# barry-mir/mixing-style-transfer

Hardware: AMD Instinct MI355X
Metric: triplets/sec (10 s @ 44.1 kHz, 4-stem, bs=24) (higher is better)
Workload: dtype f32

## Files before the change

include/mst.h:

```cpp
#ifndef MST_H_
#define MST_H_

#include <stddef.h>
#include <stdint.h>

#ifdef __cplusplus
extern "C" {
#endif

#define MST_ABI_VERSION 1

#define MST_OK 0
#define MST_EINVAL (-1)
#define MST_ENOMEM (-2)
#define MST_EHIP (-3)

int mst_version(void);
const char* mst_last_error(void);

typedef struct mst_plan mst_plan;

int mst_plan_create(mst_plan** out, int sample_rate, int n_fft, int hop, int n_mels,
                    const float* window, const float* fb, int detailed_bins);
void mst_plan_destroy(mst_plan* plan);
// ... 69 lines not shown
int mst_encoder_forward(const mst_encoder* enc, const float* logmel, int frames, const float* feats,
                        int B, float* emb, const mst_encoder_taps* taps, void* workspace,
                        size_t workspace_bytes, void* stream);

typedef struct mst_logmel_in {
  int32_t layout;
  int32_t pad_;
  const void* data;
  const void* lo;
  const uint32_t* absmax;
} mst_logmel_in;
int mst_encoder_layout_supported(const mst_encoder* enc, int layout);
int mst_encoder_forward_in(const mst_encoder* enc, const mst_logmel_in* logmel, int frames, const float* feats,
                           int B, float* emb, const mst_encoder_taps* taps, void* workspace,
                           size_t workspace_bytes, void* stream);

typedef struct mst_encoder_train_taps {
  float* film;
  float* pool1;
  float* pool_in;
  float* bn1;
  float* bn2;
  const float* film_in;
  const unsigned char* drop1_mask;
  float drop1_scale;
  int phase;
  double count_scale;
  unsigned char* drop1_mask_out;
  uint64_t drop1_seed;
  float drop1_p;
// ... 294 lines not shown
```

mixing-style-transfer_amd/_lib.py:

```python
import ctypes as C
import os
import subprocess
import threading

_HERE = os.path.dirname(os.path.abspath(__file__))
LIB_PATH = os.environ.get("MST_LIB", os.path.join(_HERE, "libmst.so"))
CSRC = os.path.join(_HERE, "csrc")

MST_OK = 0


class MstError(RuntimeError):
    pass


class EncoderConfig(C.Structure):
    _fields_ = [("n_mels", C.c_int32), ("split_size", C.c_int32), ("overlap", C.c_int32),
                ("n_subbands", C.c_int32), ("feature_dim", C.c_int32), ("embed_dim", C.c_int32),
                ("film_hidden", C.c_int32), ("attn_hidden", C.c_int32), ("bn_eps", C.c_float)]


_W_FIELDS = ["conv1_w", "conv1_b", "bn1_w", "bn1_b", "bn1_mean", "bn1_var",
             "conv2_w", "conv2_b", "bn2_w", "bn2_b", "bn2_mean", "bn2_var",
             "mlp0_w", "mlp0_b", "mlp3_w", "mlp3_b", "head_w", "head_b",
# ... 125 lines not shown
    "mst_melfeat_forward_stems_pcm16": (C.c_int, [C.c_void_p, C.POINTER(C.c_void_p), C.c_longlong, C.c_int, C.c_int,
                                                  C.c_void_p, C.c_void_p, C.c_void_p, C.c_size_t, C.c_void_p]),
    "mst_plan_layout_supported": (C.c_int, [C.c_void_p, C.c_int]),
    "mst_melfeat_forward_io": (C.c_int, [C.c_void_p, C.POINTER(MelfeatIO), C.c_int, C.c_int, C.c_void_p, C.c_size_t,
                                         C.c_void_p]),
    "mst_encoder_layout_supported": (C.c_int, [C.c_void_p, C.c_int]),
    "mst_encoder_forward_in": (C.c_int, [C.c_void_p, C.POINTER(LogmelIn), C.c_int, C.c_void_p, C.c_int, C.c_void_p,
                                         C.POINTER(EncoderTaps), C.c_void_p, C.c_size_t, C.c_void_p]),
    "mst_encoder_create": (C.c_int, [C.POINTER(C.c_void_p), C.POINTER(EncoderConfig), C.POINTER(EncoderWeights)]),
    "mst_encoder_destroy": (None, [C.c_void_p]),
    "mst_encoder_set_precision": (C.c_int, [C.c_void_p, C.c_int]),
    "mst_encoder_set_train_precision": (C.c_int, [C.c_void_p, C.c_int]),
    "mst_encoder_workspace_bytes": (C.c_size_t, [C.c_void_p, C.c_int, C.c_int]),
    "mst_encoder_forward": (C.c_int, [C.c_void_p, C.c_void_p, C.c_int, C.c_void_p, C.c_int, C.c_void_p,
                                      C.POINTER(EncoderTaps), C.c_void_p, C.c_size_t, C.c_void_p]),
    "mst_encoder_train_workspace_bytes": (C.c_size_t, [C.c_void_p, C.c_int, C.c_int]),
    "mst_encoder_forward_train": (C.c_int, [C.c_void_p, C.c_void_p, C.c_int, C.c_void_p, C.c_int, C.c_void_p,
                                            C.POINTER(EncoderTrainTaps), C.c_void_p, C.c_size_t, C.c_void_p]),
    "mst_dropout_mask": (C.c_int, [C.c_float, C.c_uint64, C.c_longlong, C.c_void_p, C.c_void_p]),
    "mst_head_save_bytes": (C.c_size_t, [C.POINTER(HeadDims), C.c_int, C.c_float]),
    "mst_head_backward_workspace_bytes": (C.c_size_t, [C.POINTER(HeadDims), C.c_int]),
    "mst_head_forward_train": (C.c_int, [C.POINTER(HeadDims), C.POINTER(HeadPtrs), C.c_void_p, C.c_int, C.c_float, C.c_uint64, C.c_float,
                                         C.c_uint64, C.c_void_p, C.c_void_p, C.c_size_t, C.c_void_p]),
    "mst_head_backward": (C.c_int, [C.POINTER(HeadDims), C.POINTER(HeadPtrs), C.c_void_p, C.c_int, C.c_float, C.c_uint64, C.c_float,
                                    C.c_uint64, C.c_void_p, C.c_void_p, C.POINTER(HeadPtrs), C.c_void_p, C.c_void_p, C.c_size_t, C.c_void_p]),
    "mst_film_save_bytes": (C.c_size_t, [C.POINTER(FilmDims), C.c_int]),
    "mst_film_backward_workspace_bytes": (C.c_size_t, [C.POINTER(FilmDims), C.c_int]),
    "mst_film_forward_train": (C.c_int, [C.POINTER(FilmDims), C.POINTER(FilmPtrs), C.c_void_p, C.c_int, C.c_float, C.c_uint64,
                                         C.c_void_p, C.c_void_p, C.c_size_t, C.c_void_p]),
    "mst_film_backward": (C.c_int, [C.POINTER(FilmDims), C.POINTER(FilmPtrs), C.c_void_p, C.c_int, C.c_float, C.c_void_p, C.c_void_p,
# ... 165 lines not shown
```

mixing-style-transfer_amd/csrc/encoder.hip:

```cpp
#include "common.h"

#include <cmath>
#include <type_traits>
#include <vector>

namespace {

typedef float f32x4 __attribute__((ext_vector_type(4)));
constexpr int kConvThreads = 512;
constexpr int kConvWaves = 8;

struct FilmParams {
  const float* feats;
  const float *w0t, *b0, *w3t, *b3, *hwt, *hb;
  const float *s1, *t1, *s2, *t2;
  float* film;
  float2* aff1;
  float2* aff2;
  int Fd, H, nsub;
  float* h2;
  int B;
};

constexpr int kFilmCT = 8;
// ... 87 lines not shown
  }
  __syncthreads();
  for (int idx = tid; idx < kFilmCT * 32; idx += 256) {
    const int c = idx >> 5, ch = idx & 31, b = b0 + c;
    if (b >= p.B) continue;
    const float g = fl[c * 64 + ch], be = fl[c * 64 + 32 + ch];
    if (slice == 0) {
      p.aff1[((size_t)b * p.nsub + band) * 32 + ch] = make_float2(g * p.s1[band * 32 + ch], fmaf(g, p.t1[band * 32 + ch], be));
    } else {
      const int c2 = 32 * (slice - 1) + ch;
      p.aff2[((size_t)b * p.nsub + band) * 64 + c2] = make_float2(g * p.s2[band * 64 + c2], fmaf(g, p.t2[band * 64 + c2], be));
    }
  }
}

constexpr size_t film_lds_bytes(int Fd, int H) {
  return (size_t)((Fd + H) * kFilmCT + 5 * kFilmCT * 64) * sizeof(float);
}
hipError_t launch_film(const FilmParams& fp, hipStream_t st) {
  const int tiles = (fp.B + kFilmCT - 1) / kFilmCT;
  const size_t lds_h = (size_t)((fp.Fd + fp.H) * kFilmCT + 4 * kFilmCT * 64) * sizeof(float);
  const size_t lds_o = (size_t)(fp.H * kFilmCT + 5 * kFilmCT * 64) * sizeof(float);
  hipLaunchKernelGGL(film_hidden_kernel, dim3(tiles, (fp.H + 63) / 64), dim3(256), lds_h, st, fp);
  hipLaunchKernelGGL(film_head_kernel, dim3(tiles, fp.nsub * 3), dim3(256), lds_o, st, fp);
  return hipGetLastError();
}

template <int LAYER, int SUB>
struct CC;
template <int SUB>
struct CC<1, SUB> {
  static constexpr int CIN = 8, COUT = 32, NCH = 2, MT = 5, NT = 2;
  static constexpr int WIN = 5 * SUB;
  static constexpr int WPG = 20 / WIN;
  static constexpr int TROWS = SUB, TCOLS = 5 * 4 * WPG;
  static constexpr int PR = TROWS + 6, PC = TCOLS + 6;
  static constexpr int RL = PC <= 64 ? 64 : 128;
};
template <int SUB>
// ... 2115 lines not shown
      for (int w = 0; w < 4; ++w)
        q4[w] = w == wave ? own[n][r] : red[((size_t)(wave * 3 + (w < wave ? w : w - 1)) * kAttnNT + n) * 256 + r * 64 + lane];
      part[r] = fmaf(w2, tanhf((q4[0] + q4[1]) + (q4[2] + q4[3]) + b1), part[r]);
    }
  }
#pragma unroll
  for (int r = 0; r < 4; ++r) {
    float v = part[r];
#pragma unroll
    for (int o = 8; o > 0; o >>= 1) v += __shfl_xor(v, o, 64);
    const int m = (mb * kAttnMT + wave) * 16 + 4 * kq + r;
    if (i == 0 && m < M) p.part[(size_t)nh * M + m] = v;
  }
}

struct PoolParams {
  const float* x;
  const float* part;
  const float* b2;
  float* pooled;
  int C, W;
  long long M;
};

__global__ __launch_bounds__(256) void attn_pool_kernel(const PoolParams p) {
  extern __shared__ float sm[];
  float* w = sm;
  __shared__ float red[8];
  const int b = blockIdx.x, tid = threadIdx.x, lane = tid & 63, wave = tid >> 6;
  const float b2 = p.b2[0];
// ... 62 lines not shown
#pragma unroll
    for (int u = 0; u < kProjU; ++u) acc = __builtin_amdgcn_mfma_f32_16x16x4f32(a[u], bb[u], acc, 0, 0, 0);
  }
#pragma unroll
  for (int r = 0; r < 4; ++r) red[wave][r][lane] = acc[r];
  __syncthreads();
  if (wave < 4) {
    const int e = nt * 16 + i, m = m0 + 4 * kq + wave;
    float v = 0.f;
#pragma unroll
    for (int w = 0; w < 8; ++w) v += red[w][wave][lane];
    if (m < p.B) p.emb[(size_t)m * p.E + e] = fmaxf(v + p.bias[e], 0.f);
  }
}

hipError_t launch_attn_scores(const AttnParams& ap, hipStream_t st) {
  const int mblocks = (ap.B * ap.W + 16 * kAttnMT - 1) / (16 * kAttnMT);
  return mst::launch_lds<attn_scores_kernel>(dim3(mblocks, kAttnHalves), dim3(256), kAttnLds, st, ap);
}

void launch_proj(const ProjParams& pj, hipStream_t st) {
  hipLaunchKernelGGL(proj_kernel, dim3(pj.E / 16, (pj.B + 15) / 16), dim3(512), 0, st, pj);
}

}

constexpr int kGenCols = 8, kGenPC = 5 * kGenCols + 6;
constexpr size_t conv1_generic_lds(int split_size) {
  return (size_t)(392 * 32 + 8 * (split_size + 6) * kGenPC) * sizeof(float);
}
__global__ __launch_bounds__(256) void conv1_generic_kernel(const ConvParams p, int sub) {
  extern __shared__ __attribute__((aligned(16))) float gsm[];
  float* wl = gsm;
  float* patch = gsm + 392 * 32;
  const int tid = threadIdx.x, co = tid & 31, pwl = tid >> 5;
  const int clip = blockIdx.y / p.nsub, band = blockIdx.y - clip * p.nsub;
  const int pw0 = blockIdx.x * kGenCols, PR = p.in_rows + 6;
// ... 1088 lines not shown
  p.in_clipstride = (long long)8 * e->cfg.n_mels * frames;
}
template <class P>
void conv2_input_geometry(P& p, const mst_encoder* e, int W1) {
  p.in_rows = e->H1, p.in_cols = W1;
  p.in_cstride = e->H1 * W1;
  p.in_bandoff = 32 * e->H1 * W1;
  p.in_clipstride = (long long)e->cfg.n_subbands * 32 * e->H1 * W1;
}

FilmParams film_params(const mst_encoder* e, const float* feats, float* film, float2* aff1, float2* aff2, float* h2, int B) {
  return FilmParams{feats, e->w0t, e->b0, e->w3t, e->b3, e->hwt, e->hb, e->s1, e->t1, e->s2, e->t2,
                    film, aff1, aff2, e->cfg.feature_dim, e->cfg.film_hidden, e->cfg.n_subbands, h2, B};
}

int launch_head(const mst_encoder* e, const WsLayout& L, char* ws, const float* pool_in, float* emb, int B, hipStream_t st,
                void* scored = nullptr) {
  float* scores = reinterpret_cast<float*>(ws + L.scores);
  AttnParams ap{pool_in, e->att0frag, e->att0_b, e->att2_w, scores, B, e->C, L.W2, e->cfg.attn_hidden};
  MST_HIP_CHECK(launch_attn_scores(ap, st));
  if (scored) (void)hipEventRecord(reinterpret_cast<hipEvent_t>(scored), st);
  float* pooled = reinterpret_cast<float*>(ws + L.pooled);
  PoolParams pp{pool_in, scores, e->att2_b, pooled, e->C, L.W2, (long long)B * L.W2};
  const int slices = (e->C + 127) / 128;
  hipLaunchKernelGGL(attn_pool_kernel, dim3(B, slices), dim3(256), (size_t)((L.W2 + 3) & ~3) * sizeof(float), st, pp);
  MST_HIP_CHECK(hipGetLastError());
  ProjParams pj{pooled, e->projfrag, e->proj_b, emb, B, e->C, e->cfg.embed_dim};
  launch_proj(pj, st);
  MST_HIP_CHECK(hipGetLastError());
  return MST_OK;
}

#ifdef MST_TRACE
struct ConvTrace {
  float* buf = nullptr;
  int calls = 0;
};
void trace_attach(ConvTrace& t, ConvParams& cp) {
  if (!t.buf) (void)hipMalloc(&t.buf, 256 * kConvWaves * 8 * sizeof(float));
  cp.yraw = t.buf;
}
void trace_dump(ConvTrace& t, int g, bool conv2) {
  if (++t.calls != 10) return;
  (void)hipDeviceSynchronize();
  std::vector<float> h(256 * kConvWaves * 8);
// ... 121 lines not shown
}

static bool conv1_resident_geometry(const mst_encoder* e) {
  return (e->sub == 2 || (e->sub == 1 && e->cfg.split_size % 2 == 0)) && !getenv("MST_CONV1_CHUNKED");
}

int mst_encoder_layout_supported(const mst_encoder* e, int layout) {
  if (!e) return 0;
  if (layout == MST_LOGMEL_REF) return 1;
  if (e->sub > 2) return 0;
  if (layout == MST_LOGMEL_CM32) return e->conv1_f16x3 == 0 && conv1_resident_geometry(e);
  if (layout == MST_LOGMEL_CM16) return e->conv1_f16x3 != 0;
  return 0;
}

int mst_encoder_forward(const mst_encoder* e, const float* logmel, int frames, const float* feats, int B, float* emb,
                        const mst_encoder_taps* taps, void* workspace, size_t workspace_bytes, void* stream) {
  mst_logmel_in in{};
  in.layout = MST_LOGMEL_REF, in.data = logmel;
  return mst_encoder_forward_in(e, &in, frames, feats, B, emb, taps, workspace, workspace_bytes, stream);
}

int mst_encoder_forward_in(const mst_encoder* e, const mst_logmel_in* lin, int frames, const float* feats, int B, float* emb,
                           const mst_encoder_taps* taps, void* workspace, size_t workspace_bytes, void* stream) {
  MST_REQUIRE(e && lin && lin->data && feats && emb, "mst_encoder_forward: NULL argument");
  const int lay = lin->layout;
  if (const int rc = check_logmel_in("mst_encoder_forward", lin, mst_encoder_layout_supported(e, lay), e->conv1_f16x3,
                                     e->conv1_f16x3 != 3, e->conv1_f16x3 >= 2))
    return rc;
  const float* logmel = static_cast<const float*>(lin->data);
// ... 1006 lines not shown
```

mixing-style-transfer_amd/csrc/infonce.hip:

```cpp
#include "common.h"

namespace {

__global__ __launch_bounds__(256) void l2norm_kernel(const float* emb, float* inv_norm, int D) {
  __shared__ float red[4];
  const int r = blockIdx.x, tid = threadIdx.x;
  float a = 0.f;
  for (int d = tid; d < D; d += 256) {
    const float v = emb[(size_t)r * D + d];
    a = fmaf(v, v, a);
  }
  a = mst::wave_sum(a);
  if ((tid & 63) == 0) red[tid >> 6] = a;
  __syncthreads();
  if (tid == 0) inv_norm[r] = 1.0f / fmaxf(sqrtf((red[0] + red[1]) + (red[2] + red[3])), 1e-12f);
}

constexpr int kInfoThreads = 512, kInfoWaves = kInfoThreads / 64;
__global__ __launch_bounds__(kInfoThreads) void infonce_fwd_kernel(const float* __restrict__ emb, const int64_t* __restrict__ labels,
                                                                   float* sim, int N, int D, int row0, float inv_tau, float* rowout) {
  extern __shared__ float srow[];
  __shared__ float red[3 * kInfoWaves];
  const int i = row0 + blockIdx.x, tid = threadIdx.x, lane = tid & 63, wave = tid >> 6;
  auto inv_of = [](float sumsq) { return 1.0f / fmaxf(sqrtf(sumsq), 1e-12f); };
  {
    float q = 0.f;
    for (int d = lane; d < D; d += 64) {
      const float v = emb[(size_t)i * D + d];
      q = fmaf(v, v, q);
    }
    const float ni = inv_of(mst::wave_sum(q));
    for (int d = tid; d < D; d += kInfoThreads) srow[d] = emb[(size_t)i * D + d] * ni;
  }
  __syncthreads();
  float* s = sim + (size_t)blockIdx.x * N;
  float mx = -INFINITY;
  for (int j0 = wave * 4; j0 < N; j0 += 4 * kInfoWaves) {
    float a[4] = {0.f, 0.f, 0.f, 0.f}, q[4] = {0.f, 0.f, 0.f, 0.f};
    const float* ej[4];
#pragma unroll
    for (int u = 0; u < 4; ++u) ej[u] = emb + (size_t)min(j0 + u, N - 1) * D;
#pragma unroll 4
    for (int d = lane; d < D; d += 64) {
      const float x = srow[d];
#pragma unroll
      for (int u = 0; u < 4; ++u) {
        const float v = ej[u][d];
        a[u] = fmaf(x, v, a[u]);
        q[u] = fmaf(v, v, q[u]);
      }
    }
#pragma unroll
    for (int u = 0; u < 4; ++u) {
      const int j = j0 + u;
      if (j >= N) break;
      const float v = mst::wave_sum(a[u]) * inv_of(mst::wave_sum(q[u])) * inv_tau;
      if (lane == 0) s[j] = v;
// ... 146 lines not shown
  return mst::align_up((size_t)N * sizeof(float), 256) + mst::align_up((size_t)N * N * sizeof(float), 256) +
         mst::align_up((size_t)2 * N * sizeof(float), 256);
}

int mst_infonce_forward(const float* emb, const int64_t* labels, int N, int D, int row0, int rows, float temperature,
                        float* out, void* workspace, size_t workspace_bytes, void* stream) {
  MST_REQUIRE(emb && labels && out, "mst_infonce_forward: NULL argument");
  MST_REQUIRE(N > 0 && D > 0 && row0 >= 0 && rows > 0 && row0 + rows <= N && temperature > 0.f,
              "mst_infonce_forward: bad sizes N=%d D=%d row0=%d rows=%d", N, D, row0, rows);
  const size_t need = mst_infonce_workspace_bytes(N, D);
  if (!workspace || workspace_bytes < need)
    return mst::fail(MST_ENOMEM, "mst_infonce_forward: workspace %zu B < required %zu B", workspace_bytes, need);
  hipStream_t st = reinterpret_cast<hipStream_t>(stream);
  float* sim = reinterpret_cast<float*>(reinterpret_cast<char*>(workspace) + mst::align_up((size_t)N * sizeof(float), 256));
  float* rowout = reinterpret_cast<float*>(reinterpret_cast<char*>(sim) + mst::align_up((size_t)N * N * sizeof(float), 256));
  hipLaunchKernelGGL(infonce_fwd_kernel, dim3(rows), dim3(kInfoThreads), (size_t)D * sizeof(float), st, emb, labels, sim, N, D, row0,
                     1.0f / temperature, rowout);
  hipLaunchKernelGGL(infonce_reduce_kernel, dim3(1), dim3(256), 0, st, rowout, rows, out);
  MST_HIP_CHECK(hipGetLastError());
  return MST_OK;
}

int mst_infonce_backward(const float* emb, const int64_t* labels, int N, int D, int row0, int rows, float temperature,
                         const float* scale, float* grad, void* workspace, size_t workspace_bytes, void* stream) {
  MST_REQUIRE(emb && labels && grad, "mst_infonce_backward: NULL argument");
  MST_REQUIRE(N > 0 && D > 0 && row0 >= 0 && rows > 0 && row0 + rows <= N && temperature > 0.f,
              "mst_infonce_backward: bad sizes N=%d D=%d row0=%d rows=%d", N, D, row0, rows);
  const size_t coef_lds = (size_t)((D + 1) & ~1) * sizeof(float) + (size_t)N * sizeof(double);
  MST_REQUIRE(coef_lds <= 64 * 1024, "mst_infonce_backward: 4 D + 8 N = %zu B of LDS, limit 65536 (N=%d D=%d)", coef_lds, N, D);
  const size_t need = mst_infonce_workspace_bytes(N, D);
  if (!workspace || workspace_bytes < need)
    return mst::fail(MST_ENOMEM, "mst_infonce_backward: workspace %zu B < required %zu B", workspace_bytes, need);
// ... 13 lines not shown
```

mixing-style-transfer_amd/csrc/melfeat.hip:

```cpp
#include "common.h"
#include "fft_wave.h"
#include "fft_pk.h"
#include "stage_a_tables.h"

#include <algorithm>
#include <cmath>
#include <memory>
#include <vector>


namespace {

constexpr int kWaves = 8;
constexpr int kFPW = 2;
constexpr int kTF = kWaves * kFPW;
constexpr int kTileStride = kTF + 1;
constexpr int kThreads = kWaves * 64;
constexpr int nf_of(int n_fft) { return n_fft >= 2048 ? 1 : kFPW; }
constexpr int kNumScalars = 80;

enum : int {
  S_LOGSUM = 0,
  S_LINSUM = 4,
  S_MASK = 8,
// ... 814 lines not shown
  double sxy = 0, sxx = 0, syy = 0;
  for (int i = lane; i < n; i += 64) {
    const double dx = i - mx, dy = y[i] - my;
    sxy += dx * dy, sxx += dx * dx, syy += dy * dy;
  }
  sxy = wave_sum_f64(sxy), sxx = wave_sum_f64(sxx), syy = wave_sum_f64(syy);
  const double std_unbiased = sqrt(syy / (n - 1));
  if (std_unbiased < 1e-6) return 0.0;
  double c = sxy / sqrt(sxx * syy);
  return fmin(1.0, fmax(-1.0, c));
}

struct FinalizeLds {
  static constexpr int a_sc = 0, a_chmean = a_sc + kNumScalars * 8, a_chm2 = a_chmean + 64, a_cross = a_chm2 + 64, a_curve = a_cross + 64;
  static constexpr size_t bytes(int M, int detailed_bins) { return (size_t)4 * M * 8 + a_curve + (size_t)4 * (detailed_bins > 0 ? detailed_bins : 0) * 8; }
};

__global__ __launch_bounds__(256) void melfeat_finalize_kernel(const FParams p) {
  extern __shared__ __attribute__((aligned(16))) unsigned char smem[];
  using L = FinalizeLds;
  double* band = reinterpret_cast<double*>(smem);
  unsigned char* after_band = reinterpret_cast<unsigned char*>(band + 4 * p.M);
  double* sc = reinterpret_cast<double*>(after_band + L::a_sc);
  double* chmean = reinterpret_cast<double*>(after_band + L::a_chmean);
  double* chm2 = reinterpret_cast<double*>(after_band + L::a_chm2);
  double* cross = reinterpret_cast<double*>(after_band + L::a_cross);
  const int tid = threadIdx.x, clip = blockIdx.x, M = p.M;
  const float* base = p.partials + (size_t)clip * p.runs_per_clip * p.pstride;
  const double inv_n_db = 1.0 / (2.0 * p.F);
  const double k_db = 10.0 / log(10.0);
  for (int i = tid; i < 4 * M; i += 256) {
    double s = 0;
#pragma unroll 8
    for (int r = 0; r < p.runs_per_clip; ++r) s += base[(size_t)r * p.pstride + i];
    band[i] = s * inv_n_db * k_db;
  }
  if (tid < kNumScalars) {
    const bool is_max = tid >= S_PEAK && tid < S_PEAK + 8;
    double s = 0;
#pragma unroll 8
    for (int r = 0; r < p.runs_per_clip; ++r) {
      const double v = base[(size_t)r * p.pstride + 4 * M + tid];
      s = is_max ? fmax(s, v) : s + v;
    }
    sc[tid] = s;
  }
  if (tid < 8) {
    double n = 0, mean = 0, m2 = 0;
    for (int r = 0; r < p.runs_per_clip; ++r) {
      const float* q = base + (size_t)r * p.pstride + 4 * M;
      const double nr = q[S_NSAMP];
      if (nr <= 0) continue;
      const double sr = q[S_DSUM + tid], qr = q[S_DSQ + tid];
      const double mr = q[S_PIVOT + tid] + sr / nr, m2r = fmax(0.0, qr - sr * sr / nr);
      const double d = mr - mean, nt = n + nr;
      m2 += m2r + d * d * n * nr / nt;
      mean += d * nr / nt;
      n = nt;
    }
    chmean[tid] = mean, chm2[tid] = m2;
  } else if (tid >= 64 && tid < 68) {
    const int s = tid - 64;
// ... 333 lines not shown
    MST_HIP_CHECK(hipMemsetAsync(lmo.absmax, 0, (size_t)B * sizeof(unsigned), st));
  }
  const int runs = use_sw ? sw_runs(p, F) : runs_per_clip(p, F);
  auto common = [&](auto k) {
    for (int i = 0; i < 4; ++i) k.stem[i] = stems4[i];
    k.clip_stride = clip_stride, k.logmel = logmel, k.partials = reinterpret_cast<float*>(workspace), k.window = p->window.get();
    k.B = B, k.T = T, k.F = F, k.M = p->n_mels, k.runs_per_clip = runs, k.pstride = pstride_of(p);
    return k;
  };
  const int rc = !use_sw            ? launch_generic_or_spw(p, common(KParams{}), pcm16, env, st)
                 : p->n_fft == 2048 ? launch_v2_2048(p, common(K4Params{}), lmo, pcm16, st)
                                    : launch_v2(p, common(K2Params{}), lmo, pcm16, env.v2_nostd, st);
  if (rc) return rc;
  if (feats) {
    const FParams fp{reinterpret_cast<const float*>(workspace), feats, p->n_mels, F, T, runs, pstride_of(p), p->detailed_bins, p->feat_dim};
    hipLaunchKernelGGL(melfeat_finalize_kernel, dim3(B), dim3(256), FinalizeLds::bytes(p->n_mels, p->detailed_bins), st, fp);
    const hipError_t e = hipGetLastError();
    if (e != hipSuccess) return mst::fail(MST_EHIP, "melfeat_finalize_kernel launch failed: %s", hipGetErrorString(e));
  }
  return MST_OK;
}

}

extern "C" {

int mst_melfeat_forward(const mst_plan* p, const float* stems, int B, int T, float* logmel, float* feats,
                        void* workspace, size_t workspace_bytes, void* stream) {
  MST_REQUIRE(p && stems, "mst_melfeat_forward: NULL plan/stems");
  const void* four[4] = {stems, stems + 2 * (size_t)T, stems + 4 * (size_t)T, stems + 6 * (size_t)T};
  return melfeat_forward_impl(p, four, false, (long long)8 * T, B, T, logmel, feats, workspace, workspace_bytes, stream);
// ... 49 lines not shown
```

mixing-style-transfer_amd/model.py:

```python
import ctypes as C

import os
import warnings

import torch
import torch.nn as nn
import torch.nn.functional as F

from . import _lib
from ._mlp import DISC, FILM, _HipMLP, _seed64, mlp_buffer, mlp_call, mlp_dims, mlp_ptrs
from .mixing_utils import (LOGMEL_BAND_MAX, STEMS, LogMel, MelFeatPlan, detailed_bins_for_feature_dim, hann_window, is_deferred,
                           feature_grad_refusal, mel_band_table, mel_bin_ranges, melfeat_backward, melscale_fbanks_htk,
                           stems_to_tensor)


class _Buf(nn.Module):
    def __init__(self, name, value):
        super().__init__()
        self.register_buffer(name, value)


class _MelTransform(nn.Module):

    def __init__(self, sample_rate, n_fft, n_mels):
# ... 589 lines not shown
            H1, W1 = self.split // sub, Fr // 5
            out = dict(film=torch.empty(B, self.n_sub * 192, device=logmel.device),
                       pool1=torch.empty(B, self.n_sub, 32, H1, W1, device=logmel.device),
                       pool_in=torch.empty(B, 64 * self.n_sub * self.freq_dim, W1 // 4, device=logmel.device))
            t = C.byref(_lib.EncoderTaps(out["film"].data_ptr(), out["pool1"].data_ptr(), out["pool_in"].data_ptr()))
        elif events is not None:
            tp = _lib.EncoderTaps()
            for i, ev in enumerate(events):
                tp.events[i] = ev.cuda_event
            t = C.byref(tp)
        with torch.cuda.device(logmel.device):
            _lib.check(L.mst_encoder_forward_in(self._h, C.byref(lin), Fr, _lib.dptr(feats.contiguous().float()), B,
                                                _lib.dptr(emb), t, _lib.dptr(self._ws), need,
                                                _lib.stream_ptr(logmel.device)), "mst_encoder_forward_in")
        return (emb, out) if taps else emb


class DistSync:

    def __init__(self, group=None):
        import torch.distributed as dist
        self._dist, self.group, self.world = dist, group, dist.get_world_size(group)

    def sum(self, t):
        self._dist.all_reduce(t, op=self._dist.ReduceOp.SUM, group=self.group)

    def max(self, t):
        self._dist.all_reduce(t, op=self._dist.ReduceOp.MAX, group=self.group)


# ... 583 lines not shown
```

Measured before the change: 2847.

## Add register-resident FiLM, attention-score, pool, projection and finalize kernel variants

Adds new kernel variants for several tail stages. FiLM hidden and head layers now keep their weights in registers, and attention scores use a buffer-load ring-pipelined MFMA kernel. Attention pooling caches activations in registers, and a projection kernel gets double-buffered loads. Melfeat finalize now parallelizes its per-run variance merge in LDS, and the InfoNCE unroll is widened. It also exposes standalone film/head forward entry points, with an env var to fall back to the old kernels. The aim is to cut latency in many small memory-bound tail kernels, at the cost of more register pressure and code complexity.

```diff
diff --git a/include/mst.h b/include/mst.h
--- a/include/mst.h
+++ b/include/mst.h
@@ -107,6 +107,11 @@
 int mst_encoder_forward_in(const mst_encoder* enc, const mst_logmel_in* logmel, int frames, const float* feats,
                            int B, float* emb, const mst_encoder_taps* taps, void* workspace,
                            size_t workspace_bytes, void* stream);
+
+int mst_encoder_film_forward(const mst_encoder* enc, const float* feats, int B, float* film, float* aff1, float* aff2,
+                             float* h2, void* stream);
+int mst_encoder_head_forward(const mst_encoder* enc, const float* pool_in, int B, int W2, float* scores, float* pooled,
+                             float* emb, void* stream);
 
 typedef struct mst_encoder_train_taps {
   float* film;
diff --git a/mixing-style-transfer_amd/_lib.py b/mixing-style-transfer_amd/_lib.py
--- a/mixing-style-transfer_amd/_lib.py
+++ b/mixing-style-transfer_amd/_lib.py
@@ -163,6 +163,10 @@
     "mst_encoder_workspace_bytes": (C.c_size_t, [C.c_void_p, C.c_int, C.c_int]),
     "mst_encoder_forward": (C.c_int, [C.c_void_p, C.c_void_p, C.c_int, C.c_void_p, C.c_int, C.c_void_p,
                                       C.POINTER(EncoderTaps), C.c_void_p, C.c_size_t, C.c_void_p]),
+    "mst_encoder_film_forward": (C.c_int, [C.c_void_p, C.c_void_p, C.c_int, C.c_void_p, C.c_void_p, C.c_void_p, C.c_void_p,
+                                           C.c_void_p]),
+    "mst_encoder_head_forward": (C.c_int, [C.c_void_p, C.c_void_p, C.c_int, C.c_int, C.c_void_p, C.c_void_p, C.c_void_p,
+                                           C.c_void_p]),
     "mst_encoder_train_workspace_bytes": (C.c_size_t, [C.c_void_p, C.c_int, C.c_int]),
     "mst_encoder_forward_train": (C.c_int, [C.c_void_p, C.c_void_p, C.c_int, C.c_void_p, C.c_int, C.c_void_p,
                                             C.POINTER(EncoderTrainTaps), C.c_void_p, C.c_size_t, C.c_void_p]),
diff --git a/mixing-style-transfer_amd/csrc/encoder.hip b/mixing-style-transfer_amd/csrc/encoder.hip
--- a/mixing-style-transfer_amd/csrc/encoder.hip
+++ b/mixing-style-transfer_amd/csrc/encoder.hip
@@ -125,15 +125,137 @@
   }
 }
 
+constexpr int kFilmKQ = 64, kFilmKQ0 = 16, kFilmPasses = 4;
+
+template <int KQ>
+__device__ __forceinline__ void film_fetch(const float* __restrict__ wt, int K, int N, int j, int kq, float (&w)[KQ]) {
+  const int kper = (K + 3) / 4, k0 = kq * kper;
+  const float* wp = wt + min(j, N - 1);
+#pragma unroll
+  for (int u = 0; u < KQ; ++u) w[u] = wp[(size_t)min(k0 + u, K - 1) * N];
+}
+template <int KQ>
+__device__ __forceinline__ void film_dot_regs(const float (&w)[KQ], int K, int N, int j, const float* hin, int kq, float (&acc)[kFilmCT]) {
+#pragma unroll
+  for (int c = 0; c < kFilmCT; ++c) acc[c] = 0.f;
+  if (j >= N) return;
+  const int kper = (K + 3) / 4, k0 = kq * kper, k1 = min(K, k0 + kper);
+#pragma unroll
+  for (int u = 0; u < KQ; ++u) {
+    const int i = k0 + u;
+    if (i < k1) {
+      const float4 ha = *reinterpret_cast<const float4*>(hin + i * kFilmCT), hb = *reinterpret_cast<const float4*>(hin + i * kFilmCT + 4);
+      acc[0] = fmaf(w[u], ha.x, acc[0]), acc[1] = fmaf(w[u], ha.y, acc[1]), acc[2] = fmaf(w[u], ha.z, acc[2]), acc[3] = fmaf(w[u], ha.w, acc[3]);
+      acc[4] = fmaf(w[u], hb.x, acc[4]), acc[5] = fmaf(w[u], hb.y, acc[5]), acc[6] = fmaf(w[u], hb.z, acc[6]), acc[7] = fmaf(w[u], hb.w, acc[7]);
+    }
+  }
+}
+
+__global__ __launch_bounds__(256) void film_hidden_regs_kernel(const FilmParams p) {
+  extern __shared__ __attribute__((aligned(16))) float sm[];
+  float* f = sm;
+  float* h1 = f + p.Fd * kFilmCT;
+  float* red = h1 + p.H * kFilmCT;
+  const int tid = threadIdx.x, jl = tid & 63, kq = tid >> 6;
+  const int b0 = blockIdx.x * kFilmCT;
+  const int j = blockIdx.y * 64 + jl;
+  float w0[kFilmPasses][kFilmKQ0], w3[kFilmKQ];
+#pragma unroll
+  for (int q = 0; q < kFilmPasses; ++q) film_fetch(p.w0t, p.Fd, p.H, q * 64 + jl, kq, w0[q]);
+  film_fetch(p.w3t, p.H, p.H, j, kq, w3);
+  for (int idx = tid; idx < p.Fd * kFilmCT; idx += 256) {
+    const int c = idx / p.Fd, i = idx % p.Fd;
+    f[i * kFilmCT + c] = b0 + c < p.B ? p.feats[(size_t)(b0 + c) * p.Fd + i] : 0.f;
+  }
+  __syncthreads();
+  float acc[kFilmCT], out[2];
+#pragma unroll
+  for (int q = 0; q < kFilmPasses; ++q) {
+    const int j0 = q * 64;
+    if (j0 >= p.H) break;
+    film_dot_regs(w0[q], p.Fd, p.H, j0 + jl, f, kq, acc);
+    film_reduce(red, acc, jl, kq, out);
+    if (j0 + jl < p.H) {
+      const float bias = p.b0[j0 + jl];
+      h1[(j0 + jl) * kFilmCT + kq] = fmaxf(out[0] + bias, 0.f);
+      h1[(j0 + jl) * kFilmCT + kq + 4] = fmaxf(out[1] + bias, 0.f);
+    }
+    __syncthreads();
+  }
+  film_dot_regs(w3, p.H, p.H, j, h1, kq, acc);
+  film_reduce(red, acc, jl, kq, out);
+  if (j < p.H) {
+    const float bias = p.b3[j];
+#pragma unroll
+    for (int r = 0; r < 2; ++r)
+      if (b0 + kq + 4 * r < p.B) p.h2[(size_t)(b0 + kq + 4 * r) * p.H + j] = fmaxf(out[r] + bias, 0.f);
+  }
+}
+
+__global__ __launch_bounds__(256) void film_head_regs_kernel(const FilmParams p) {
+  extern __shared__ __attribute__((aligned(16))) float sm[];
+  float* h2 = sm;
+  float* red = h2 + p.H * kFilmCT;
+  float* fl = red + 4 * kFilmCT * 64;
+  const int tid = threadIdx.x, jl = tid & 63, kq = tid >> 6;
+  const int b0 = blockIdx.x * kFilmCT;
+  const int band = blockIdx.y / 3, slice = blockIdx.y % 3;
+  const int nout = p.nsub * 192;
+  const int col = slice == 0 ? jl : (jl < 32 ? 32 + 32 * slice + jl : 96 + 32 * slice + (jl - 32));
+  const int o = band * 192 + col;
+  float hw[kFilmKQ];
+  film_fetch(p.hwt, p.H, nout, o, kq, hw);
+  const float bias = p.hb[o];
+  for (int idx = tid; idx < p.H * kFilmCT; idx += 256) {
+    const int c = idx / p.H, i = idx % p.H;
+    h2[i * kFilmCT + c] = b0 + c < p.B ? p.h2[(size_t)(b0 + c) * p.H + i] : 0.f;
+  }
+  __syncthreads();
+  float acc[kFilmCT], out[2];
+  film_dot_regs(hw, p.H, nout, o, h2, kq, acc);
+  film_reduce(red, acc, jl, kq, out);
+#pragma unroll
+  for (int r = 0; r < 2; ++r) {
+    const int c = kq + 4 * r;
+    const float v = out[r] + bias;
+    fl[c * 64 + jl] = v;
+    if (b0 + c < p.B) p.film[(size_t)(b0 + c) * nout + o] = v;
+  }
+  __syncthreads();
+  for (int idx = tid; idx < kFilmCT * 32; idx += 256) {
+    const int c = idx >> 5, ch = idx & 31, b = b0 + c;
+    if (b >= p.B) continue;
+    const float g = fl[c * 64 + ch], be = fl[c * 64 + 32 + ch];
+    if (slice == 0) {
+      p.aff1[((size_t)b * p.nsub + band) * 32 + ch] = make_float2(g * p.s1[band * 32 + ch], fmaf(g, p.t1[band * 32 + ch], be));
+    } else {
+      const int c2 = 32 * (slice - 1) + ch;
+      p.aff2[((size_t)b * p.nsub + band) * 64 + c2] = make_float2(g * p.s2[band * 64 + c2], fmaf(g, p.t2[band * 64 + c2], be));
+    }
+  }
+}
+
 constexpr size_t film_lds_bytes(int Fd, int H) {
   return (size_t)((Fd + H) * kFilmCT + 5 * kFilmCT * 64) * sizeof(float);
 }
+bool tail_parent() {
+  const char* env = getenv("MST_TAIL_KERNELS");
+  return env && !strcmp(env, "parent");
+}
+
 hipError_t launch_film(const FilmParams& fp, hipStream_t st) {
   const int tiles = (fp.B + kFilmCT - 1) / kFilmCT;
   const size_t lds_h = (size_t)((fp.Fd + fp.H) * kFilmCT + 4 * kFilmCT * 64) * sizeof(float);
   const size_t lds_o = (size_t)(fp.H * kFilmCT + 5 * kFilmCT * 64) * sizeof(float);
-  hipLaunchKernelGGL(film_hidden_kernel, dim3(tiles, (fp.H + 63) / 64), dim3(256), lds_h, st, fp);
-  hipLaunchKernelGGL(film_head_kernel, dim3(tiles, fp.nsub * 3), dim3(256), lds_o, st, fp);
+  const bool parent = tail_parent();
+  if (!parent && fp.H <= 4 * kFilmKQ && fp.H <= 64 * kFilmPasses && fp.Fd <= 4 * kFilmKQ0)
+    hipLaunchKernelGGL(film_hidden_regs_kernel, dim3(tiles, (fp.H + 63) / 64), dim3(256), lds_h, st, fp);
+  else
+    hipLaunchKernelGGL(film_hidden_kernel, dim3(tiles, (fp.H + 63) / 64), dim3(256), lds_h, st, fp);
+  if (!parent && fp.H <= 4 * kFilmKQ)
+    hipLaunchKernelGGL(film_head_regs_kernel, dim3(tiles, fp.nsub * 3), dim3(256), lds_o, st, fp);
+  else
+    hipLaunchKernelGGL(film_head_kernel, dim3(tiles, fp.nsub * 3), dim3(256), lds_o, st, fp);
   return hipGetLastError();
 }
 
@@ -2279,6 +2401,124 @@
   }
 }
 
+template <int MT>
+constexpr size_t attn_ring_lds() { return (size_t)4 * 3 * kAttnNT * MT * 64 * sizeof(float); }
+
+template <int MT, int U, int R>
+__global__ __launch_bounds__(256, MT == 2 ? 2 : 1) void attn_scores_ring_kernel(const AttnParams p) {
+  extern __shared__ float red[];
+  const int lane = threadIdx.x & 63;
+  const int wave = __builtin_amdgcn_readfirstlane(threadIdx.x >> 6);
+  const int l = blockIdx.x;
+  const int mb = (l >> 4) * 8 + (l & 7), nh = (l >> 3) & 1;
+  const int M = p.B * p.W;
+  if (mb * MT * 16 >= M) return;
+  const int kq = lane >> 4, i = lane & 15;
+  const __amdgpu_buffer_rsrc_t xr =
+      __builtin_amdgcn_make_buffer_rsrc(const_cast<float*>(p.x), 0, (unsigned)((size_t)M * p.C * sizeof(float)), 0x00020000);
+  const __amdgpu_buffer_rsrc_t wr =
+      __builtin_amdgcn_make_buffer_rsrc(const_cast<float*>(p.w1frag), 0, (unsigned)((size_t)p.C * 256 * sizeof(float)), 0x00020000);
+  unsigned xo[MT];
+#pragma unroll
+  for (int q = 0; q < MT; ++q) {
+    const int m = min((mb * MT + q) * 16 + i, M - 1);
+    xo[q] = (unsigned)(((m / p.W) * p.C + kq) * p.W + m % p.W) * 4u;
+  }
+  const unsigned wo = (unsigned)(nh * kAttnNT * 64 + lane) * 4u;
+  const unsigned xstep = (unsigned)(4 * p.W) * 4u, wstep = 16u * 64u * 4u;
+  f32x4 acc[MT][kAttnNT];
+#pragma unroll
+  for (int q = 0; q < MT; ++q)
+#pragma unroll
+    for (int n = 0; n < kAttnNT; ++n) acc[q][n] = f32x4{0.f, 0.f, 0.f, 0.f};
+  const int steps = p.C / 4;
+  const int s0 = wave * steps / 4, s1 = (wave + 1) * steps / 4;
+  const int nb = (s1 - s0 + U - 1) / U;
+  float a[R][U][MT], bb[R][U][kAttnNT];
+  auto load_batch = [&](int j, int buf) __attribute__((always_inline)) {
+#pragma unroll
+    for (int u = 0; u < U; ++u) {
+      const unsigned s = (unsigned)min(s0 + j * U + u, s1 - 1);
+#pragma unroll
+      for (int q = 0; q < MT; ++q) a[buf][u][q] = __builtin_bit_cast(float, __builtin_amdgcn_raw_buffer_load_b32(xr, xo[q], s * xstep, 0));
+#pragma unroll
+      for (int n = 0; n < kAttnNT; ++n)
+        bb[buf][u][n] = __builtin_bit_cast(float, __builtin_amdgcn_raw_buffer_load_b32(wr, wo + (unsigned)n * 256u, s * wstep, 0));
+    }
+  };
+  auto mfma_batch = [&](int j, int buf) __attribute__((always_inline)) {
+#pragma unroll
+    for (int u = 0; u < U; ++u) {
+      const bool live = s0 + j * U + u < s1;
+#pragma unroll
+      for (int q = 0; q < MT; ++q) {
+        const float av = live ? a[buf][u][q] : 0.f;
+#pragma unroll
+        for (int n = 0; n < kAttnNT; ++n) acc[q][n] = __builtin_amdgcn_mfma_f32_16x16x4f32(av, bb[buf][u][n], acc[q][n], 0, 0, 0);
+      }
+    }
+  };
+  if (s0 < s1) {
+#pragma unroll
+    for (int r = 0; r < R - 1; ++r) {
+      load_batch(r, r);
+      __builtin_amdgcn_sched_barrier(0);
+    }
+    for (int j = 0; j < nb; j += R) {
+#pragma unroll
+      for (int r = 0; r < R; ++r) {
+        load_batch(j + r + R - 1, (r + R - 1) % R);
+        if (j + r < nb) mfma_batch(j + r, r);
+      }
+    }
+  }
+  const int oq = wave % MT, oh = wave / MT;
+  float own[kAttnNT][MT];
+#pragma unroll
+  for (int q = 0; q < MT; ++q)
+#pragma unroll
+    for (int h = 0; h < 4 / MT; ++h) {
+      const int d = q + MT * h;
+      if (d == wave) {
+#pragma unroll
+        for (int n = 0; n < kAttnNT; ++n)
+#pragma unroll
+          for (int r = 0; r < MT; ++r) own[n][r] = acc[q][n][MT * h + r];
+      } else {
+        float* dst = red + ((size_t)(d * 3 + (wave < d ? wave : wave - 1)) * kAttnNT) * (MT * 64) + lane;
+#pragma unroll
+        for (int n = 0; n < kAttnNT; ++n)
+#pragma unroll
+          for (int r = 0; r < MT; ++r) dst[n * (MT * 64) + r * 64] = acc[q][n][MT * h + r];
+      }
+    }
+  __syncthreads();
+  float part[MT];
+#pragma unroll
+  for (int r = 0; r < MT; ++r) part[r] = 0.f;
+#pragma unroll
+  for (int n = 0; n < kAttnNT; ++n) {
+    const int h = (nh * kAttnNT + n) * 16 + i;
+    const float w2 = p.w2[h], b1 = p.b1[h];
+#pragma unroll
+    for (int r = 0; r < MT; ++r) {
+      float q4[4];
+#pragma unroll
+      for (int w = 0; w < 4; ++w)
+        q4[w] = w == wave ? own[n][r] : red[((size_t)(wave * 3 + (w < wave ? w : w - 1)) * kAttnNT + n) * (MT * 64) + r * 64 + lane];
+      part[r] = fmaf(w2, tanhf((q4[0] + q4[1]) + (q4[2] + q4[3]) + b1), part[r]);
+    }
+  }
+#pragma unroll
+  for (int r = 0; r < MT; ++r) {
+    float v = part[r];
+#pragma unroll
+    for (int o = 8; o > 0; o >>= 1) v += __shfl_xor(v, o, 64);
+    const int m = (mb * MT + oq) * 16 + 4 * kq + MT * oh + r;
+    if (i == 0 && m < M) p.part[(size_t)nh * M + m] = v;
+  }
+}
+
 struct PoolParams {
   const float* x;
   const float* part;
@@ -2371,13 +2611,136 @@
   }
 }
 
+template <int MT, int U, int R>
+hipError_t launch_attn_ring(const AttnParams& ap, hipStream_t st) {
+  const int mblocks = (ap.B * ap.W + 16 * MT - 1) / (16 * MT);
+  return mst::launch_lds<attn_scores_ring_kernel<MT, U, R>>(dim3((mblocks + 7) / 8 * 16), dim3(256), attn_ring_lds<MT>(), st, ap);
+}
+
 hipError_t launch_attn_scores(const AttnParams& ap, hipStream_t st) {
+  const char* env = getenv("MST_ATTN_SCORES");
+  const bool fits = (size_t)ap.B * ap.W * ap.C * sizeof(float) < ((size_t)1 << 31);
+  if (fits && !(env && !strcmp(env, "64x128"))) {
+    if (env && !strcmp(env, "ring")) return launch_attn_ring<4, 2, 4>(ap, st);
+    return launch_attn_ring<2, 2, 4>(ap, st);
+  }
   const int mblocks = (ap.B * ap.W + 16 * kAttnMT - 1) / (16 * kAttnMT);
   return mst::launch_lds<attn_scores_kernel>(dim3(mblocks, kAttnHalves), dim3(256), kAttnLds, st, ap);
 }
 
+constexpr int kPoolT = 6, kPoolP = 8;
+__global__ __launch_bounds__(256) void attn_pool_regs_kernel(const PoolParams p) {
+  extern __shared__ float sm[];
+  float* w = sm;
+  __shared__ float red[8];
+  const int b = blockIdx.x, tid = threadIdx.x, lane = tid & 63, wave = tid >> 6;
+  const int c_per_blk = (p.C + gridDim.y - 1) / gridDim.y;
+  const int c0 = blockIdx.y * c_per_blk, c1 = min(p.C, c0 + c_per_blk);
+  const float* xb = p.x + (size_t)b * p.C * p.W;
+  const int sub = lane >> 4, l16 = lane & 15;
+  float xv[kPoolP][kPoolT];
+#pragma unroll
+  for (int q = 0; q < kPoolP; ++q) {
+    const float* xc = xb + (size_t)min(c0 + wave * 4 + sub + 16 * q, c1 - 1) * p.W;
+#pragma unroll
+    for (int k = 0; k < kPoolT; ++k) xv[q][k] = xc[min(l16 + 16 * k, p.W - 1)];
+  }
+  const float b2 = p.b2[0];
+  float mx = -INFINITY;
+  for (int t = tid; t < p.W; t += 256) {
+    const float s = (p.part[(size_t)b * p.W + t] + p.part[(size_t)p.M + (size_t)b * p.W + t]) + b2;
+    w[t] = s;
+    mx = fmaxf(mx, s);
+  }
+  mx = mst::wave_max(mx);
+  if (lane == 0) red[wave] = mx;
+  __syncthreads();
+  mx = fmaxf(fmaxf(red[0], red[1]), fmaxf(red[2], red[3]));
+  float sum = 0.f;
+  for (int t = tid; t < p.W; t += 256) {
+    const float e = expf(w[t] - mx);
+    w[t] = e;
+    sum += e;
+  }
+  sum = mst::wave_sum(sum);
+  if (lane == 0) red[4 + wave] = sum;
+  __syncthreads();
+  const float inv = 1.0f / ((red[4] + red[5]) + (red[6] + red[7]));
+  float wl[kPoolT];
+#pragma unroll
+  for (int k = 0; k < kPoolT; ++k) wl[k] = l16 + 16 * k < p.W ? w[l16 + 16 * k] * inv : 0.f;
+#pragma unroll
+  for (int q = 0; q < kPoolP; ++q) {
+    const int c = c0 + wave * 4 + sub + 16 * q;
+    float v = 0.f;
+#pragma unroll
+    for (int k = 0; k < kPoolT; ++k)
+      if (l16 + 16 * k < p.W) v = fmaf(xv[q][k], wl[k], v);
+#pragma unroll
+    for (int o = 8; o > 0; o >>= 1) v += __shfl_xor(v, o, 64);
+    if (l16 == 0 && c < c1) p.pooled[(size_t)b * p.C + c] = v;
+  }
+}
+
+constexpr int kProjPipeU = 16;
+__global__ __launch_bounds__(512) void proj_pipe_kernel(const ProjParams p) {
+  __shared__ float red[8][4][64];
+  const int lane = threadIdx.x & 63, wave = __builtin_amdgcn_readfirstlane(threadIdx.x >> 6);
+  const int nt = blockIdx.x, NTE = p.E / 16;
+  const int kq = lane >> 4, i = lane & 15;
+  const int m0 = blockIdx.y * 16;
+  f32x4 acc = f32x4{0.f, 0.f, 0.f, 0.f};
+  const float* ap = p.pooled + (size_t)min(m0 + i, p.B - 1) * p.C + kq;
+  const float* wf = p.wfrag + (size_t)nt * 64 + lane;
+  const int steps = p.C / 4;
+  const int s0 = wave * steps / 8, s1 = (wave + 1) * steps / 8;
+  float bb[2][kProjPipeU], a[2][kProjPipeU];
+  auto load_batch = [&](int sb, int buf) __attribute__((always_inline)) {
+#pragma unroll
+    for (int u = 0; u < kProjPipeU; ++u) {
+      const int s = min(sb + u, s1 - 1);
+      bb[buf][u] = wf[(size_t)s * NTE * 64];
+      a[buf][u] = ap[4 * s];
+    }
+  };
+  auto mfma_batch = [&](int sb, int buf) __attribute__((always_inline)) {
+#pragma unroll
+    for (int u = 0; u < kProjPipeU; ++u)
+      acc = __builtin_amdgcn_mfma_f32_16x16x4f32(a[buf][u], sb + u < s1 ? bb[buf][u] : 0.f, acc, 0, 0, 0);
+  };
+  if (s0 < s1) {
+    load_batch(s0, 0);
+    for (int sb = s0; sb < s1; sb += 2 * kProjPipeU) {
+      if (sb + kProjPipeU < s1) load_batch(sb + kProjPipeU, 1);
+      mfma_batch(sb, 0);
+      if (sb + 2 * kProjPipeU < s1) load_batch(sb + 2 * kProjPipeU, 0);
+      if (sb + kProjPipeU < s1) mfma_batch(sb + kProjPipeU, 1);
+    }
+  }
+#pragma unroll
+  for (int r = 0; r < 4; ++r) red[wave][r][lane] = acc[r];
+  __syncthreads();
+  if (wave < 4) {
+    const int e = nt * 16 + i, m = m0 + 4 * kq + wave;
+    float v = 0.f;
+#pragma unroll
+    for (int w = 0; w < 8; ++w) v += red[w][wave][lane];
+    if (m < p.B) p.emb[(size_t)m * p.E + e] = fmaxf(v + p.bias[e], 0.f);
+  }
+}
+
+hipError_t launch_attn_pool(const PoolParams& pp, int B, hipStream_t st) {
+  const int slices = (pp.C + 127) / 128;
+  const size_t lds = (size_t)((pp.W + 3) & ~3) * sizeof(float);
+  if (pp.W <= 16 * kPoolT && !tail_parent()) hipLaunchKernelGGL(attn_pool_regs_kernel, dim3(B, slices), dim3(256), lds, st, pp);
+  else hipLaunchKernelGGL(attn_pool_kernel, dim3(B, slices), dim3(256), lds, st, pp);
+  return hipGetLastError();
+}
+
 void launch_proj(const ProjParams& pj, hipStream_t st) {
-  hipLaunchKernelGGL(proj_kernel, dim3(pj.E / 16, (pj.B + 15) / 16), dim3(512), 0, st, pj);
+  const dim3 grid(pj.E / 16, (pj.B + 15) / 16);
+  if (tail_parent()) hipLaunchKernelGGL(proj_kernel, grid, dim3(512), 0, st, pj);
+  else hipLaunchKernelGGL(proj_pipe_kernel, grid, dim3(512), 0, st, pj);
 }
 
 }
@@ -3496,21 +3859,22 @@
                     film, aff1, aff2, e->cfg.feature_dim, e->cfg.film_hidden, e->cfg.n_subbands, h2, B};
 }
 
-int launch_head(const mst_encoder* e, const WsLayout& L, char* ws, const float* pool_in, float* emb, int B, hipStream_t st,
-                void* scored = nullptr) {
-  float* scores = reinterpret_cast<float*>(ws + L.scores);
-  AttnParams ap{pool_in, e->att0frag, e->att0_b, e->att2_w, scores, B, e->C, L.W2, e->cfg.attn_hidden};
+int launch_head_on(const mst_encoder* e, const float* pool_in, int B, int W2, float* scores, float* pooled, float* emb,
+                   hipStream_t st, void* scored = nullptr) {
+  AttnParams ap{pool_in, e->att0frag, e->att0_b, e->att2_w, scores, B, e->C, W2, e->cfg.attn_hidden};
   MST_HIP_CHECK(launch_attn_scores(ap, st));
   if (scored) (void)hipEventRecord(reinterpret_cast<hipEvent_t>(scored), st);
-  float* pooled = reinterpret_cast<float*>(ws + L.pooled);
-  PoolParams pp{pool_in, scores, e->att2_b, pooled, e->C, L.W2, (long long)B * L.W2};
-  const int slices = (e->C + 127) / 128;
-  hipLaunchKernelGGL(attn_pool_kernel, dim3(B, slices), dim3(256), (size_t)((L.W2 + 3) & ~3) * sizeof(float), st, pp);
-  MST_HIP_CHECK(hipGetLastError());
+  PoolParams pp{pool_in, scores, e->att2_b, pooled, e->C, W2, (long long)B * W2};
+  MST_HIP_CHECK(launch_attn_pool(pp, B, st));
   ProjParams pj{pooled, e->projfrag, e->proj_b, emb, B, e->C, e->cfg.embed_dim};
   launch_proj(pj, st);
   MST_HIP_CHECK(hipGetLastError());
   return MST_OK;
+}
+int launch_head(const mst_encoder* e, const WsLayout& L, char* ws, const float* pool_in, float* emb, int B, hipStream_t st,
+                void* scored = nullptr) {
+  return launch_head_on(e, pool_in, B, L.W2, reinterpret_cast<float*>(ws + L.scores), reinterpret_cast<float*>(ws + L.pooled), emb,
+                        st, scored);
 }
 
 #ifdef MST_TRACE
@@ -3662,6 +4026,21 @@
   return 0;
 }
 
+int mst_encoder_film_forward(const mst_encoder* e, const float* feats, int B, float* film, float* aff1, float* aff2, float* h2,
+                             void* stream) {
+  MST_REQUIRE(e && feats && film && aff1 && aff2 && h2 && B > 0, "mst_encoder_film_forward: NULL / bad argument");
+  MST_HIP_CHECK(launch_film(film_params(e, feats, film, reinterpret_cast<float2*>(aff1), reinterpret_cast<float2*>(aff2), h2, B),
+                            reinterpret_cast<hipStream_t>(stream)));
+  return MST_OK;
+}
+
+int mst_encoder_head_forward(const mst_encoder* e, const float* pool_in, int B, int W2, float* scores, float* pooled, float* emb,
+                             void* stream) {
+  MST_REQUIRE(e && pool_in && scores && pooled && emb && B > 0 && W2 > 0, "mst_encoder_head_forward: NULL / bad argument");
+  MST_REQUIRE((size_t)W2 * sizeof(float) <= 48 * 1024, "mst_encoder_head_forward: W2 = %d: the pooling kernel keeps a clip's scores in LDS", W2);
+  return launch_head_on(e, pool_in, B, W2, scores, pooled, emb, reinterpret_cast<hipStream_t>(stream));
+}
+
 int mst_encoder_forward(const mst_encoder* e, const float* logmel, int frames, const float* feats, int B, float* emb,
                         const mst_encoder_taps* taps, void* workspace, size_t workspace_bytes, void* stream) {
   mst_logmel_in in{};
diff --git a/mixing-style-transfer_amd/csrc/infonce.hip b/mixing-style-transfer_amd/csrc/infonce.hip
--- a/mixing-style-transfer_amd/csrc/infonce.hip
+++ b/mixing-style-transfer_amd/csrc/infonce.hip
@@ -17,6 +17,7 @@
 }
 
 constexpr int kInfoThreads = 512, kInfoWaves = kInfoThreads / 64;
+template <int DU>
 __global__ __launch_bounds__(kInfoThreads) void infonce_fwd_kernel(const float* __restrict__ emb, const int64_t* __restrict__ labels,
                                                                    float* sim, int N, int D, int row0, float inv_tau, float* rowout) {
   extern __shared__ float srow[];
@@ -25,6 +26,7 @@
   auto inv_of = [](float sumsq) { return 1.0f / fmaxf(sqrtf(sumsq), 1e-12f); };
   {
     float q = 0.f;
+#pragma unroll DU
     for (int d = lane; d < D; d += 64) {
       const float v = emb[(size_t)i * D + d];
       q = fmaf(v, v, q);
@@ -40,7 +42,7 @@
     const float* ej[4];
 #pragma unroll
     for (int u = 0; u < 4; ++u) ej[u] = emb + (size_t)min(j0 + u, N - 1) * D;
-#pragma unroll 4
+#pragma unroll DU
     for (int d = lane; d < D; d += 64) {
       const float x = srow[d];
 #pragma unroll
@@ -217,8 +219,13 @@
   hipStream_t st = reinterpret_cast<hipStream_t>(stream);
   float* sim = reinterpret_cast<float*>(reinterpret_cast<char*>(workspace) + mst::align_up((size_t)N * sizeof(float), 256));
   float* rowout = reinterpret_cast<float*>(reinterpret_cast<char*>(sim) + mst::align_up((size_t)N * N * sizeof(float), 256));
-  hipLaunchKernelGGL(infonce_fwd_kernel, dim3(rows), dim3(kInfoThreads), (size_t)D * sizeof(float), st, emb, labels, sim, N, D, row0,
-                     1.0f / temperature, rowout);
+  const char* tail = getenv("MST_TAIL_KERNELS");
+  if (tail && !strcmp(tail, "parent"))
+    hipLaunchKernelGGL(infonce_fwd_kernel<4>, dim3(rows), dim3(kInfoThreads), (size_t)D * sizeof(float), st, emb, labels, sim, N, D, row0,
+                       1.0f / temperature, rowout);
+  else
+    hipLaunchKernelGGL(infonce_fwd_kernel<12>, dim3(rows), dim3(kInfoThreads), (size_t)D * sizeof(float), st, emb, labels, sim, N, D, row0,
+                       1.0f / temperature, rowout);
   hipLaunchKernelGGL(infonce_reduce_kernel, dim3(1), dim3(256), 0, st, rowout, rows, out);
   MST_HIP_CHECK(hipGetLastError());
   return MST_OK;
diff --git a/mixing-style-transfer_amd/csrc/melfeat.hip b/mixing-style-transfer_amd/csrc/melfeat.hip
--- a/mixing-style-transfer_amd/csrc/melfeat.hip
+++ b/mixing-style-transfer_amd/csrc/melfeat.hip
@@ -852,8 +852,11 @@
 struct FinalizeLds {
   static constexpr int a_sc = 0, a_chmean = a_sc + kNumScalars * 8, a_chm2 = a_chmean + 64, a_cross = a_chm2 + 64, a_curve = a_cross + 64;
   static constexpr size_t bytes(int M, int detailed_bins) { return (size_t)4 * M * 8 + a_curve + (size_t)4 * (detailed_bins > 0 ? detailed_bins : 0) * 8; }
+  static constexpr int kParPerRun = 42;
+  static constexpr size_t bytes_par(int M, int detailed_bins, int runs) { return bytes(M, detailed_bins) + (size_t)kParPerRun * runs * 8; }
 };
 
+template <bool PAR>
 __global__ __launch_bounds__(256) void melfeat_finalize_kernel(const FParams p) {
   extern __shared__ __attribute__((aligned(16))) unsigned char smem[];
   using L = FinalizeLds;
@@ -867,23 +870,92 @@
   const float* base = p.partials + (size_t)clip * p.runs_per_clip * p.pstride;
   const double inv_n_db = 1.0 / (2.0 * p.F);
   const double k_db = 10.0 / log(10.0);
+  constexpr int kRunUnroll = PAR ? 32 : 8;
   for (int i = tid; i < 4 * M; i += 256) {
     double s = 0;
-#pragma unroll 8
+#pragma unroll kRunUnroll
     for (int r = 0; r < p.runs_per_clip; ++r) s += base[(size_t)r * p.pstride + i];
     band[i] = s * inv_n_db * k_db;
   }
   if (tid < kNumScalars) {
     const bool is_max = tid >= S_PEAK && tid < S_PEAK + 8;
     double s = 0;
-#pragma unroll 8
+#pragma unroll kRunUnroll
     for (int r = 0; r < p.runs_per_clip; ++r) {
       const double v = base[(size_t)r * p.pstride + 4 * M + tid];
       s = is_max ? fmax(s, v) : s + v;
     }
     sc[tid] = s;
   }
-  if (tid < 8) {
+  if constexpr (PAR) {
+    const int R = p.runs_per_clip;
+    double* mr = reinterpret_cast<double*>(after_band + L::a_curve) + 4 * (p.detailed_bins > 0 ? p.detailed_bins : 0);
+    double* m2r = mr + 8 * R;
+    double* dd = m2r + 8 * R;
+    double* nrs = dd + 8 * R;
+    double* nbef = nrs + R;
+    double* cr = nbef + R;
+    double* term = cr + 4 * R;
+    for (int idx = tid; idx < 8 * R; idx += 256) {
+      const int r = idx >> 3, c = idx & 7;
+      const float* q = base + (size_t)r * p.pstride + 4 * M;
+      const double nr = q[S_NSAMP];
+      if (c == 0) nrs[r] = nr;
+      const double sr = q[S_DSUM + c], qr = q[S_DSQ + c], pv = q[S_PIVOT + c];
+      if (nr <= 0) continue;
+      mr[c * R + r] = pv + sr / nr, m2r[c * R + r] = fmax(0.0, qr - sr * sr / nr);
+    }
+    for (int idx = tid; idx < 4 * R; idx += 256) {
+      const int r = idx >> 2, s = idx & 3;
+      const float* q = base + (size_t)r * p.pstride + 4 * M;
+      const double nr = q[S_NSAMP];
+      const double sL = q[S_DSUM + 2 * s], sR = q[S_DSUM + 2 * s + 1], cs = q[S_CROSS + s];
+      if (nr <= 0) continue;
+      cr[s * R + r] = cs - sL * sR / nr;
+    }
+    __syncthreads();
+    if (tid < 8) {
+      double n = 0, mean = 0;
+#pragma unroll 4
+      for (int r = 0; r < R; ++r) {
+        const double nr = nrs[r], m = mr[tid * R + r];
+        if (tid == 0) nbef[r] = n;
+        if (nr <= 0) continue;
+        const double d = m - mean, nt = n + nr;
+        dd[tid * R + r] = d;
+        mean += d * nr / nt;
+        n = nt;
+      }
+      chmean[tid] = mean;
+    }
+    __syncthreads();
+    for (int idx = tid; idx < 12 * R; idx += 256) {
+      const int r = idx / 12, k = idx % 12;
+      const double nr = nrs[r];
+      if (nr <= 0) continue;
+      const double n = nbef[r], nt = n + nr;
+      if (k < 8) {
+        const double d = dd[k * R + r];
+        term[k * R + r] = m2r[k * R + r] + d * d * n * nr / nt;
+      } else {
+        const int s = k - 8;
+        const double dL = dd[2 * s * R + r], dR = dd[(2 * s + 1) * R + r];
+        term[k * R + r] = cr[s * R + r] + dL * dR * n * nr / nt;
+      }
+    }
+    __syncthreads();
+    if (tid < 12) {
+      double a = 0;
+#pragma unroll 4
+      for (int r = 0; r < R; ++r) {
+        const double t = term[tid * R + r];
+        if (nrs[r] <= 0) continue;
+        a += t;
+      }
+      if (tid < 8) chm2[tid] = a;
+      else cross[tid - 8] = a;
+    }
+  } else if (tid < 8) {
     double n = 0, mean = 0, m2 = 0;
     for (int r = 0; r < p.runs_per_clip; ++r) {
       const float* q = base + (size_t)r * p.pstride + 4 * M;
@@ -1247,7 +1319,12 @@
   if (rc) return rc;
   if (feats) {
     const FParams fp{reinterpret_cast<const float*>(workspace), feats, p->n_mels, F, T, runs, pstride_of(p), p->detailed_bins, p->feat_dim};
-    hipLaunchKernelGGL(melfeat_finalize_kernel, dim3(B), dim3(256), FinalizeLds::bytes(p->n_mels, p->detailed_bins), st, fp);
+    const char* tail = getenv("MST_TAIL_KERNELS");
+    const size_t lds_par = FinalizeLds::bytes_par(p->n_mels, p->detailed_bins, runs);
+    if (lds_par <= 48 * 1024 && !(tail && !strcmp(tail, "parent")))
+      hipLaunchKernelGGL(melfeat_finalize_kernel<true>, dim3(B), dim3(256), lds_par, st, fp);
+    else
+      hipLaunchKernelGGL(melfeat_finalize_kernel<false>, dim3(B), dim3(256), FinalizeLds::bytes(p->n_mels, p->detailed_bins), st, fp);
     const hipError_t e = hipGetLastError();
     if (e != hipSuccess) return mst::fail(MST_EHIP, "melfeat_finalize_kernel launch failed: %s", hipGetErrorString(e));
   }
diff --git a/mixing-style-transfer_amd/model.py b/mixing-style-transfer_amd/model.py
--- a/mixing-style-transfer_amd/model.py
+++ b/mixing-style-transfer_amd/model.py
@@ -627,6 +627,29 @@
                                                 _lib.dptr(emb), t, _lib.dptr(self._ws), need,
                                                 _lib.stream_ptr(logmel.device)), "mst_encoder_forward_in")
         return (emb, out) if taps else emb
+
+    def film_forward(self, feats):
+        feats = feats.contiguous().float()
+        B, dev = feats.shape[0], feats.device
+        film = torch.empty(B, self.n_sub * 192, device=dev)
+        aff1, aff2 = torch.empty(B, self.n_sub, 32, 2, device=dev), torch.empty(B, self.n_sub, 64, 2, device=dev)
+        h2 = torch.empty(B, self.cfg.film_hidden, device=dev)
+        with torch.cuda.device(dev):
+            _lib.check(_lib.lib().mst_encoder_film_forward(self._h, _lib.dptr(feats), B, _lib.dptr(film), _lib.dptr(aff1),
+                                                           _lib.dptr(aff2), _lib.dptr(h2), _lib.stream_ptr(dev)),
+                       "mst_encoder_film_forward")
+        return film, aff1, aff2
+
+    def head_forward(self, pool_in):
+        pool_in = pool_in.contiguous().float()
+        (B, Cc, W2), dev = pool_in.shape, pool_in.device
+        assert Cc == 64 * self.n_sub * self.freq_dim, (Cc, self.n_sub, self.freq_dim)
+        scores, pooled = torch.empty(2, B, W2, device=dev), torch.empty(B, Cc, device=dev)
+        emb = torch.empty(B, self.embed_dim, device=dev)
+        with torch.cuda.device(dev):
+            _lib.check(_lib.lib().mst_encoder_head_forward(self._h, _lib.dptr(pool_in), B, W2, _lib.dptr(scores), _lib.dptr(pooled),
+                                                           _lib.dptr(emb), _lib.stream_ptr(dev)), "mst_encoder_head_forward")
+        return scores, pooled, emb
 
 
 class DistSync:
```

After: 2852 (median of 6 runs). Within noise of the previous version (+0.2%).
